# robotic-vision-lab/Edge-Informed-Contrast-Maximization

Hardware: AMD Instinct MI355X
Metric: warped-events/sec/GPU + loss+grad eval ms, 1e6 events @ 346x260 (higher is better)
Workload: dtype f32

## Files before the change

### edge-informed-contrast-maximization_amd/csrc/eincm_api.hip

```cpp
#include <hip/hip_runtime.h>
#include <hip/hip_ext.h>

#include <algorithm>
#include <chrono>
#include <cmath>
#include <cstdarg>
#include <cstdio>
#include <cstdlib>
#include <cstring>
#include <string>
#include <vector>

#include "eincm.h"
#include "eincm_kernels.hip.h"
#include "eincm_kernels_f64.hip.h"
#include "eincm_binning.hip.h"
#include "eincm_edges.hip.h"
#include "eincm_objectives.hip.h"
#include "eincm_splat_window.hip.h"
#include "eincm_canny.hip.h"
#include "eincm_preprocess.hip.h"
#include "eincm_gtflow.hip.h"

using namespace eincm;
// ... 1236 lines not shown
    if (n_in < 1 || n_out < 1 || !A || method < 0 || method > EINCM_METHOD_CUBIC) return EINCM_ERR_ARG;
    std::vector<double> M;
    resample_matrix(n_in, n_out, method, M);
    memcpy(A, M.data(), M.size() * sizeof(double));
    return EINCM_OK;
}

eincm_ctx* eincm_create(int device, int H, int W, int max_refs, int max_windows, int64_t max_events_total, uint32_t flags) {
    if (H < 3 || W < 3 || H > 32767 || W > 32767 || max_refs < 1 || max_refs > EINCM_MAX_REFS || max_windows < 1 ||
        max_events_total < 1 || max_events_total > (int64_t)2000000000) {
        fail(nullptr, EINCM_ERR_ARG, "eincm_create: bad argument (H=%d W=%d max_refs=%d max_windows=%d max_events=%lld)",
             H, W, max_refs, max_windows, (long long)max_events_total);
        return nullptr;
    }
    int ndev = 0;
    hipError_t e = hipGetDeviceCount(&ndev);
    if (e != hipSuccess || ndev < 1) {
        fail(nullptr, EINCM_ERR_HIP, "eincm_create: no HIP device visible (%s); this engine has no CPU fallback",
             hipGetErrorString(e));
        return nullptr;
    }
    if (device < 0 || device >= ndev) {
        fail(nullptr, EINCM_ERR_ARG, "eincm_create: device %d out of range (0..%d)", device, ndev - 1);
        return nullptr;
    }
    if ((flags & EINCM_CF_FP64) && (flags & (EINCM_CF_TIMING | EINCM_CF_TIMING_DOMINANT))) {
        fail(nullptr, EINCM_ERR_UNSUPPORTED, "eincm_create: the timing flags are not supported with EINCM_CF_FP64");
        return nullptr;
    }
    eincm_ctx* c = new eincm_ctx();
    c->fp64 = (flags & EINCM_CF_FP64) != 0;
    c->device = device; c->H = H; c->W = W; c->maxR = max_refs; c->maxB = max_windows; c->maxN = max_events_total;
    c->cflags = flags;
    if (const char* s = getenv("EINCM_SEG")) { int v = atoi(s); if (v >= 64 && v <= MAX_SEG) c->seg = v; }
    if (const char* s = getenv("EINCM_SEG_SPLAT")) { int v = atoi(s); if (v >= 64 && v <= MAX_CHUNK) c->seg_s = v; }
    if (const char* s = getenv("EINCM_WINCAP")) { int v = atoi(s); if (v >= 1024 && v <= 6912) { c->wincap = (v / 4) * 4; c->wincap_fixed = true; } }
    auto bail = [&](const char* what, hipError_t err) -> eincm_ctx* {
        fail(nullptr, EINCM_ERR_HIP, "eincm_create: %s failed: %s", what, hipGetErrorString(err));
        free_all(c);
        delete c;
        return nullptr;
    };
#define TRY(expr) do { hipError_t e2_ = (expr); if (e2_ != hipSuccess) return bail(#expr, e2_); } while (0)
    TRY(hipSetDevice(device));
    TRY(hipStreamCreateWithFlags(&c->stream, hipStreamNonBlocking));
    const int tilesX = (W + TS - 1) / TS, tilesY = (H + TS - 1) / TS, ntiles = tilesX * tilesY;
    const size_t B = max_windows, R = max_refs, img = (size_t)H * W;
    c->max_items = (int64_t)B * ntiles + max_events_total / 256 + 1;
    c->coarse_cap = 64 * 64 * 2;
    TRY(dalloc(&c->d_xy, (size_t)max_events_total));
    TRY(dalloc(&c->d_t, (size_t)max_events_total));
    TRY(dalloc(&c->d_xy_g, (size_t)max_events_total));
    TRY(dalloc(&c->d_t_g, (size_t)max_events_total));
    c->host_binning = (ntiles > BIN_MAX_TILES) || (getenv("EINCM_HOST_BINNING") != nullptr);
    for (SegList* L : {&c->gather, &c->splat, &c->splat_sh, &c->gather_2}) {
        TRY(dalloc(&L->d_items, (size_t)c->max_items));
        TRY(dalloc(&L->d_order, (size_t)c->max_items));
    }
    for (SegList* L : {&c->gather, &c->gather_2}) TRY(dalloc(&L->d_win_item0, B + 1));
    for (SegList* L : {&c->gather, &c->splat}) {
        TRY(dalloc(&L->d_wins, (size_t)c->max_items * max_refs));
        if (!c->host_binning) TRY(dalloc(&L->d_itembase, B * ntiles));
    }
    TRY(dalloc(&c->d_raw_x, (size_t)max_events_total));
    TRY(dalloc(&c->d_raw_y, (size_t)max_events_total));
    TRY(dalloc(&c->d_raw_t, (size_t)max_events_total));
    if (!c->host_binning) {
// ... 153 lines not shown
    if (c && c->pend.active && c->pend.launched)
        return fail(c, EINCM_ERR_STATE, "an asynchronous evaluation is in flight: call eincm_loss_grad_wait first");
    if (!c) return EINCM_ERR_ARG;
    if (n_windows < 1 || n_windows > c->maxB) return fail(c, EINCM_ERR_ARG, "n_windows %d outside 1..%d", n_windows, c->maxB);
    if (n_refs < 1 || n_refs > c->maxR) return fail(c, EINCM_ERR_ARG, "n_refs %d outside 1..%d", n_refs, c->maxR);
    if (!n_events || !xs_w || !ys_w || !ts_w || !edges_w || !edge_ts) return fail(c, EINCM_ERR_ARG, "null pointer argument");
    if (n_windows >= 1 && n_windows <= c->maxB)
        for (int b = 0; b < n_windows; ++b)
            if (!edges_w[b] || (n_events[b] > 0 && (!xs_w[b] || !ys_w[b] || !ts_w[b]))) return fail(c, EINCM_ERR_ARG, "null pointer argument (window %d)", b);
    HIPCHK(c, hipSetDevice(c->device));
    c->objc_valid = false;
    const int H = c->H, W = c->W;
    int64_t N = 0;
    for (int b = 0; b < n_windows; ++b) {
        if (n_events[b] < 0) return fail(c, EINCM_ERR_ARG, "n_events[%d] negative", b);
        N += n_events[b];
    }
    if (N > c->maxN) return fail(c, EINCM_ERR_ARG, "total events %lld exceed capacity %lld", (long long)N, (long long)c->maxN);
    c->staged = false;
    c->Theta_valid = false;
    struct DrainOnExit { hipStream_t s; ~DrainOnExit() { (void)hipStreamSynchronize(s); } } drain_on_exit{c->stream};
    if (c->acc_dirty) { const int rcd = clear_accumulators(c); if (rcd) return rcd; }
    Geom g{};
    g.H = H; g.W = W; g.R = n_refs; g.B = n_windows;
    g.tilesX = (W + TS - 1) / TS; g.tilesY = (H + TS - 1) / TS; g.ntiles = g.tilesX * g.tilesY;
    g.igx = (W + IG_COLS - 1) / IG_COLS; g.nig = g.igx * ((H + IG_ROWS - 1) / IG_ROWS);
    g.pstride = std::max(g.ntiles, NSPART);
    g.gmax_n = g.R * g.nig;
    g.wincap = c->wincap; g.winmaxw = win_maxw(c->wincap);
    g.wincap_a = g.wincap; g.winmaxw_a = g.winmaxw;

    const double x_wg = ((double)N / 8192.0 + 0.5 * n_windows * g.ntiles) * n_refs;
    int seg = c->seg > 0 ? c->seg : 16384;
    int seg_2 = (x_wg >= 4000.0 && (double)N / ((double)n_windows * g.ntiles) < 16384.0) ? 16384 : (x_wg < 1000.0 ? 4096 : 8192);
    if (const char* e = getenv("EINCM_SEG_2DOF")) { const int v = atoi(e); if (v >= 64 && v <= MAX_SEG) seg_2 = v; }
    const double per_tile = (double)N / ((double)n_windows * g.ntiles);
    int seg_s = c->seg_s > 0 ? c->seg_s : (x_wg >= 3000.0 && per_tile < 16384.0 ? 16384 : (x_wg >= 400.0 ? 8192 : 4096));
    g.pitch_aligned = (x_wg >= 3000.0 && per_tile < 16384.0) ? 1 : 0;
    if (const char* e = getenv("EINCM_PITCH_ALIGNED")) g.pitch_aligned = std::max(0, std::min(2, atoi(e)));
    const bool sort_segments = getenv("EINCM_NO_SEGSORT") == nullptr;
    const size_t img = (size_t)H * W;
    for (int b = 0; b < n_windows; ++b) {
        memset(&c->h_wc[b], 0, sizeof(WinConst));
        multi_ref_weights(n_refs, c->h_wc[b].mrw);
        for (int r = 0; r < n_refs; ++r)
            if (!std::isfinite(edge_ts[b * n_refs + r])) return fail(c, EINCM_ERR_ARG, "edge_ts[%d,%d] is not finite", b, r);
    }
    std::vector<unsigned> cntmax_h((size_t)n_windows, 0u);
    std::vector<double> dtmax_h((size_t)n_windows, 0.0);
    bool edge_ts_uploaded = false;
    int rc = EINCM_OK;
    auto copy_for_gather = [&]() -> int {
        if (c->gather.n == 0) return EINCM_OK;
        if (sort_segments) {
            hipLaunchKernelGGL(k_segsort, dim3(std::min(c->gather.n, 8192)), dim3(SORT_NT), 0, c->stream, c->gather.n, c->gather.d_items,
                               c->d_xy, c->d_t, c->d_xy_g, c->d_t_g);
            return EINCM_OK;
        }
        HIPCHK(c, hipMemcpyAsync(c->d_xy_g, c->d_xy, (size_t)N * sizeof(uint32_t), hipMemcpyDeviceToDevice, c->stream));
        HIPCHK(c, hipMemcpyAsync(c->d_t_g, c->d_t, (size_t)N * sizeof(double), hipMemcpyDeviceToDevice, c->stream));
        return EINCM_OK;
    };
    if (!c->host_binning) {
        std::vector<BinBlock> blks;
        std::vector<int32_t> win_blk((size_t)n_windows + 1);
        int64_t base = 0;
        for (int b = 0; b < n_windows; ++b) {
            win_blk[b] = (int32_t)blks.size();
            for (int64_t s0 = 0; s0 < n_events[b]; s0 += BIN_CHUNK) {
                BinBlock bb; bb.win = b; bb.start = (int32_t)(base + s0); bb.count = (int32_t)std::min<int64_t>(BIN_CHUNK, n_events[b] - s0);
                bb.first_blk = win_blk[b];
                blks.push_back(bb);
            }
            base += n_events[b];
        }
        win_blk[n_windows] = (int32_t)blks.size();
        const int nblk = (int)blks.size();
        if (nblk > c->max_binblocks) return fail(c, EINCM_ERR_ARG, "internal: %d staging blocks exceed capacity", nblk);
        int32_t misc_init[4] = {0, 0, 0x7fffffff, 0x7fffffff};
        HIPCHK(c, hipMemcpyAsync(c->d_bin_misc, misc_init, sizeof misc_init, hipMemcpyHostToDevice, c->stream));
        HIPCHK(c, hipMemcpyAsync(c->d_win_blk, win_blk.data(), win_blk.size() * sizeof(int32_t), hipMemcpyHostToDevice, c->stream));
        for (int b = 0; b < n_windows; ++b)
            HIPCHK(c, hipMemcpyAsync(c->d_edges_raw + (size_t)b * n_refs * img, edges_w[b], (size_t)n_refs * img * sizeof(double), hipMemcpyHostToDevice, c->stream));
        hipLaunchKernelGGL(k_edges, dim3(EDGE_PARTS, n_refs, n_windows), dim3(NT), 0, c->stream, g, c->d_edges_raw, c->d_edges, c->d_edge_moments);
        if (nblk > 0) {
            HIPCHK(c, hipMemcpyAsync(c->d_binblocks, blks.data(), blks.size() * sizeof(BinBlock), hipMemcpyHostToDevice, c->stream));
            int64_t off = 0;
            for (int b = 0; b < n_windows; ++b) {
                const size_t nb = (size_t)n_events[b];
                if (nb > 0) {
                    HIPCHK(c, hipMemcpyAsync(c->d_raw_x + off, xs_w[b], nb * sizeof(int16_t), hipMemcpyHostToDevice, c->stream));
                    HIPCHK(c, hipMemcpyAsync(c->d_raw_y + off, ys_w[b], nb * sizeof(int16_t), hipMemcpyHostToDevice, c->stream));
// ... 1121 lines not shown
```

### edge-informed-contrast-maximization_amd/csrc/eincm_binning.hip.h

```cpp
#pragma once
#include <hip/hip_runtime.h>
#include <stdint.h>

#include "eincm_kernels.hip.h"

namespace eincm {

constexpr int BIN_CHUNK = 1024;
constexpr int BIN_NT = 64;
constexpr int BIN_TRIPS = BIN_CHUNK / BIN_NT;
constexpr int BIN_MAX_TILES = 12288;

struct BinBlock { int32_t win, start, count, first_blk; };

__global__ __launch_bounds__(BIN_NT) void k_bin_hist(Geom g, const BinBlock* __restrict__ blks, const int16_t* __restrict__ xs,
                                                  const int16_t* __restrict__ ys, const double* __restrict__ ts,
                                                  uint32_t* __restrict__ blockhist, int* __restrict__ err)
{
    extern __shared__ uint32_t hist[];
    const BinBlock bb = blks[blockIdx.x];
    uint32_t xy[BIN_TRIPS]; double tt[BIN_TRIPS];
#pragma unroll
    for (int k = 0; k < BIN_TRIPS; ++k) {
        const int i = k * BIN_NT + (int)threadIdx.x;
// ... 119 lines not shown
    __shared__ __attribute__((aligned(16))) uint32_t keys[256];
    const int idx = blockIdx.x;
    const int cnt = tilecount[idx], base = tilebase[idx];
    const int t = threadIdx.x;
    for (int b0 = blockIdx.y * 256; b0 + 256 <= cnt; b0 += 256 * gridDim.y) {
        const uint32_t xy = ev_xy[base + b0 + t];
        const double tm = ev_t[base + b0 + t];
        const uint32_t key = (((xy & 31u) << 5) | ((xy >> 16) & 31u)) << 8 | (uint32_t)t;
        __syncthreads();
        keys[t] = key;
        __syncthreads();
        int rank = 0;
        const uint4* k4 = reinterpret_cast<const uint4*>(keys);
#pragma unroll 8
        for (int k = 0; k < 64; ++k) {
            const uint4 q = k4[k];
            rank += (q.x < key ? 1 : 0) + (q.y < key ? 1 : 0) + (q.z < key ? 1 : 0) + (q.w < key ? 1 : 0);
        }
        const int hw = rank & 7;
        const int pos = (hw >> 1) * 64 + (hw & 1) * 32 + (rank >> 3);
        ev_xy[base + b0 + pos] = xy;
        ev_t[base + b0 + pos] = tm;
    }
}

struct SegLayout {
    int n0, K0, K1, rem0, rem1;
    __host__ __device__ explicit SegLayout(int n) {
        n0 = (n + 1) >> 1;
        const int n1 = n - n0;
        K0 = (n0 + 255) >> 8; K1 = (n1 + 255) >> 8;
        rem0 = n0 - 256 * (K0 - 1); rem1 = n1 - 256 * (K1 - 1);
    }
    __host__ __device__ int position(int s) const {
        const int c = s >= n0;
        const int sc = c ? s - n0 : s, K = c ? K1 : K0, rem = c ? rem1 : rem0;
        int t, j;
        if (sc < rem * K) { t = sc / K; j = sc - t * K; }
        else { const int q = sc - rem * K; t = rem + q / (K - 1); j = q - (t - rem) * (K - 1); }
        return (c ? n0 : 0) + j * 256 + t;
    }
};
constexpr int SORT_NT = 256, SORT_NW = SORT_NT / 64, SORT_KEYS = TS * TS, SORT_KEY_BITS = 10;
static_assert(SORT_KEYS == 1 << SORT_KEY_BITS, "pixkey has SORT_KEY_BITS bits");
__device__ __forceinline__ uint32_t pixkey(uint32_t xy) { return ((xy >> 11) & (31u << 5)) | (xy & 31u); }
__global__ __launch_bounds__(SORT_NT) void k_segsort(int n_items, const Item* __restrict__ items,
                                                      const uint32_t* __restrict__ src_xy, const double* __restrict__ src_t,
                                                      uint32_t* __restrict__ dst_xy, double* __restrict__ dst_t)
{
    __shared__ uint32_t cnt[SORT_NW][SORT_KEYS];
    __shared__ uint32_t wsum[SORT_NT];
    const int lane = threadIdx.x & 63, wv = threadIdx.x >> 6;
    const unsigned long long lt_mask = (1ull << lane) - 1ull;
    for (int k = blockIdx.x; k < n_items; k += gridDim.x) {
        const Item it = items[k];
        const int n = it.count, begin = it.begin;
        const int qlen = (((n + SORT_NW - 1) / SORT_NW + 63) / 64) * 64;
        const int lo = min(wv * qlen, n), hi = min(lo + qlen, n);
        for (int i = threadIdx.x; i < SORT_NW * SORT_KEYS; i += SORT_NT) (&cnt[0][0])[i] = 0u;
        __syncthreads();
        for (int i = lo + lane; i < hi; i += 64) atomicAdd(&cnt[wv][pixkey(src_xy[begin + i])], 1u);
        __syncthreads();
        uint32_t c[4][SORT_NW], tot = 0u;
#pragma unroll
        for (int q = 0; q < 4; ++q)
#pragma unroll
            for (int w = 0; w < SORT_NW; ++w) { c[q][w] = cnt[w][4 * threadIdx.x + q]; tot += c[q][w]; }
        wsum[threadIdx.x] = tot;
        __syncthreads();
        for (int off = 1; off < SORT_NT; off <<= 1) {
            const uint32_t v = (threadIdx.x >= off) ? wsum[threadIdx.x - off] : 0u;
            __syncthreads();
            wsum[threadIdx.x] += v;
            __syncthreads();
        }
        uint32_t run = wsum[threadIdx.x] - tot;
#pragma unroll
        for (int q = 0; q < 4; ++q)
#pragma unroll
            for (int w = 0; w < SORT_NW; ++w) { cnt[w][4 * threadIdx.x + q] = run; run += c[q][w]; }
        __syncthreads();
        const SegLayout L(n);
        uint32_t nxy = 0u; double nt = 0.0;
        if (lo + lane < hi) { nxy = src_xy[begin + lo + lane]; nt = src_t[begin + lo + lane]; }
        for (int i0 = lo; i0 < hi; i0 += 64) {
            const int i = i0 + lane;
            const bool valid = i < hi;
            const uint32_t xy = nxy; const double t = nt;
            if (i + 64 < hi) { nxy = src_xy[begin + i + 64]; nt = src_t[begin + i + 64]; }
            const int key = valid ? (int)pixkey(xy) : -1;
            unsigned long long grp = __ballot(valid);
#pragma unroll
            for (int bit = 0; bit < SORT_KEY_BITS; ++bit) {
                const bool one = ((key >> bit) & 1) != 0;
                const unsigned long long bal = __ballot(one);
                grp &= one ? bal : ~bal;
            }
            uint32_t rank = 0u, base = 0u;
            if (valid) { base = cnt[wv][key]; rank = base + (uint32_t)__popcll(grp & lt_mask); }
            __builtin_amdgcn_wave_barrier();
            if (valid && (grp & lt_mask) == 0ull) cnt[wv][key] = base + (uint32_t)__popcll(grp);
            __builtin_amdgcn_wave_barrier();
            if (valid) {
                const int pos = L.position((int)rank);
                dst_xy[begin + pos] = xy;
                dst_t[begin + pos] = t;
            }
        }
        __syncthreads();
    }
}

__global__ void k_items(Geom g, int seg, const int32_t* __restrict__ tilecount, const int32_t* __restrict__ tilebase,
                        const int32_t* __restrict__ itembase, Item* __restrict__ items)
{
    const int idx = blockIdx.x * blockDim.x + threadIdx.x;
    if (idx >= g.B * g.ntiles) return;
    const int c = tilecount[idx], base = tilebase[idx];
    int k = itembase[idx];
    const int len = balanced_seg_len(c, seg);
    for (int s = 0; s < c; s += len, ++k) {
        Item it;
        it.win = idx / g.ntiles; it.tile = idx % g.ntiles; it.begin = base + s; it.count = min(len, c - s);
        it.t_lo = 0.0; it.t_hi = 0.0;
        items[k] = it;
    }
}

__global__ __launch_bounds__(NT) void k_seg_minmax(int n_items, Item* __restrict__ items, const double* __restrict__ ev_t)
{
    __shared__ double smn[NWAVE], smx[NWAVE];
    for (int k = blockIdx.x; k < n_items; k += gridDim.x) {
        const int begin = items[k].begin, count = items[k].count;
        double mn = INFINITY, mx = -INFINITY;
        for (int i = threadIdx.x; i < count; i += NT) { const double t = ev_t[begin + i]; mn = fmin(mn, t); mx = fmax(mx, t); }
        mn = wave_min(mn); mx = wave_max(mx);
        __syncthreads();
        if ((threadIdx.x & 63) == 0) { smn[threadIdx.x >> 6] = mn; smx[threadIdx.x >> 6] = mx; }
        __syncthreads();
        if (threadIdx.x == 0) {
            for (int i = 1; i < NWAVE; ++i) { mn = fmin(mn, smn[i]); mx = fmax(mx, smx[i]); }
            items[k].t_lo = mn; items[k].t_hi = mx;
        }
// ... 54 lines not shown
```

### edge-informed-contrast-maximization_amd/csrc/eincm_kernels.hip.h

```cpp
#pragma once
#include <hip/hip_runtime.h>
#include <stdint.h>

namespace eincm {

constexpr int TS = 32;
constexpr int NT = 256;
constexpr int NWAVE = NT / 64;
constexpr int WIN_CAP_DEFAULT = 2304;
constexpr int WIN_CAP_MAX = 9216;
constexpr int NXCD = 8;
constexpr double EPSN = 2.220446049250313e-16;
constexpr float INV_2PI = 0.15915494309189535f;
constexpr int MAX_CHUNK = 16384;
constexpr int MAX_SEG = 1 << 20;
__device__ __forceinline__ int fix_shift(int count) {
    const unsigned c = (unsigned)ceilf((float)count * 0.16f);
    const int ceillog2 = (c <= 1u) ? 0 : (32 - __clz(c - 1u));
    return min(30, 32 - ceillog2);
}
__host__ __device__ __forceinline__ int balanced_seg_len(int c, int seg) {
    const int nseg = (c + seg - 1) / seg;
    if (nseg <= 1) return seg;
    const int len = (((c + nseg - 1) / nseg + 255) / 256) * 256;
    return len < seg ? len : seg;
}
constexpr float EXP_M05 = 0.6065306597126334f;

struct Geom {
    int H, W, R, B;
    int tilesX, tilesY, ntiles;
    int wincap, winmaxw;
    int wincap_a, winmaxw_a;
    int nparts;
    int pstride;
    int gmax_n;
    unsigned long long wmask;
    int igx, nig;
    int pitch_aligned;
};

__device__ __forceinline__ bool win_active(const Geom& g, int b) { return b >= 64 || ((g.wmask >> b) & 1ull) != 0ull; }

struct Item {
    int32_t win, tile, begin, count;
    double t_lo, t_hi;
};

// ... 148 lines not shown
        const int nwh = min(wh, wincap / (aligned ? win_pitch(g, nww) : nww));
        bx0 = (bx0 + bx1) / 2 - nww / 2;
        by0 = (by0 + by1) / 2 - nwh / 2;
        ww = nww; wh = nwh;
    }
    Window w; w.ox = bx0; w.oy = by0; w.ww = ww; w.wh = wh;
    return w;
}

__device__ __forceinline__ void warp_axis(int x, double v, double dt, int& ir, float& f) {
#ifndef EINCM_ABL_WARP_FMA
#pragma clang fp contract(off)
#endif
    const double w = (double)x - v * dt;
    const double r = rint(w);
    f = (float)(w - r);
    ir = (int)r;
}
__device__ __forceinline__ int clamp_far(int ir) { return min(max(ir, -(1 << 20)), 1 << 20); }

struct f2v { float x, y; };

__device__ __forceinline__ void taps3x2(float fx, float fy, float scale_y, f2v& km, f2v& k0, f2v& kp) {
    constexpr float L2E = 1.4426950408889634f, EXP_M1 = 0.36787944117144233f;
    const float bx = __builtin_amdgcn_exp2f(fmaf(fx, L2E, -0.5f * L2E)), by = __builtin_amdgcn_exp2f(fmaf(fy, L2E, -0.5f * L2E));
    const float ax = EXP_M1 * __builtin_amdgcn_rcpf(bx), ay = EXP_M1 * __builtin_amdgcn_rcpf(by);
    const float s = __builtin_amdgcn_exp2f(fmaf(fx, fx, fy * fy) * (-0.5f * L2E)) * scale_y;
    km.x = ax; km.y = s * ay;
    k0.x = 1.0f; k0.y = s;
    kp.x = bx; kp.y = s * by;
}

struct EvReg { uint32_t xy; double t; };

constexpr int THETA_CONST = 1;
constexpr int THETA_TILE = 2;

__device__ __forceinline__ uint32_t cvt_rpi(float x) { uint32_t r; asm("v_cvt_rpi_i32_f32 %0, %1" : "=v"(r) : "v"(x)); return r; }
__device__ __forceinline__ uint32_t fix_u32(float a, float b) { return cvt_rpi(a * b); }

constexpr int RS_MAXC = 24;
struct TileRange { int ilo, ni, jlo, nj; };
struct ResampleTile {
    int ilo, ni, jlo, nj;
    bool staged;
};
struct ResampleLds {
    int2 rt[TS], ct[TS];
    double ah[TS * RS_MAXC], aw[TS * RS_MAXC];
    int rng[4];
};
__device__ __forceinline__ ResampleTile stage_resample_ranges(ResampleLds& L, int h, int w, int x0, int y0, int x1, int y1,
                                                              const int2* __restrict__ rowtap, const int2* __restrict__ coltap) {
    const int t = threadIdx.x;
    if (t < TS) L.rt[t] = (y0 + t < y1) ? rowtap[y0 + t] : make_int2(h, 0);
    else if (t < 2 * TS) L.ct[t - TS] = (x0 + t - TS < x1) ? coltap[x0 + t - TS] : make_int2(w, 0);
    __syncthreads();
    if (t < 64) {
        const int2 v = (t < TS) ? L.rt[t] : L.ct[t - TS];
        int lo = v.x, hi = v.y;
#pragma unroll
        for (int o = 16; o > 0; o >>= 1) { lo = min(lo, __shfl_xor(lo, o, 64)); hi = max(hi, __shfl_xor(hi, o, 64)); }
        if (t == 0) { L.rng[0] = lo; L.rng[1] = hi; }
        if (t == TS) { L.rng[2] = lo; L.rng[3] = hi; }
    }
    __syncthreads();
// ... 983 lines not shown
        }
    }
    if (!direct11) for (int i = threadIdx.x; i < TS * TS * 2; i += NTH) accum[i] = 0ull;
    auto G_at = [&](size_t p) -> float { return Gi[p]; };
    auto load_window = [&]() {
    if (wn.ox >= 0 && wn.oy >= 0 && wn.ox + wn.ww <= g.W && wn.oy + wn.wh <= g.H) {
        const size_t o0 = (size_t)wn.oy * g.W + wn.ox;
        for (WinWalkT<NTH> w(threadIdx.x, wn.ww); w.i < wn.ww * wn.wh; w.next()) lds[w.row * wp + w.col] = G_at(o0 + w.row * g.W + w.col);
    } else {
        for (int row = wv; row < wn.wh; row += NTH / 64) {
            const int gy = wrap_drop(wn.oy + row, g.H);
            for (int col = lane; col < wn.ww; col += 64) {
                const int gx = wrap_drop(wn.ox + col, g.W);
                lds[row * wp + col] = (gx >= 0 && gy >= 0) ? G_at((size_t)gy * g.W + gx) : 0.0f;
            }
        }
    }
    };
    load_window();
    double gscale = 0.0;
    double gm_used = 0.0;
    if (!direct11) {
        __shared__ unsigned gms[NTH / 64];
        const double gm = gmax_of(gmax + (size_t)it.win * g.gmax_n, g.gmax_n, gms);
        gscale = ldexp(1.0, grad_shift_pixel(wc[it.win], gm, g.R, WIDE != 0));
        gm_used = gm;
    }
    __syncthreads();

    const uint32_t* __restrict__ exy = ev_xy + it.begin;
    const double* __restrict__ et = ev_t + it.begin;
    const int n = it.count;
    const int tid = threadIdx.x;
    uint32_t cur_key = 0xffffffffu;
    double run_x = 0.0, run_y = 0.0;
    double2 vcur = vconst;
    auto flush_run = [&]() {
        if (cur_key == 0xffffffffu) return;
        unsigned long long* a = accum + (cur_key << 1);
        atomicAdd(a, (unsigned long long)(WIDE ? fix64_wide(run_x) : fix64(run_x)));
        atomicAdd(a + 1, (unsigned long long)(WIDE ? fix64_wide(run_y) : fix64(run_y)));
    };
    auto gather_ev = [&](const EvReg& ev) {
        const double dt = ev.t - tau;
        const int x = ev.xy & 0xffff, y = ev.xy >> 16;
        if (theta_mode != THETA_CONST) {
            const uint32_t key = ((ev.xy >> 11) & (31u << 5)) | (ev.xy & 31u);
#ifdef EINCM_ABL_G_NORUN
            vcur = thtile[key];
#else
            if (key != cur_key) {
                flush_run();
                cur_key = key; run_x = 0.0; run_y = 0.0;
                vcur = thtile[key];
            }
#endif
        }
        float gwx, gwy;
        event_dLdw(g, wn, wp, lds, G_at, x, y, vcur, dt, gwx, gwy);
        if (direct11) {
            const float ndt = (float)(-dt);
            f11x = fmaf(ndt, gwx, f11x); f11y = fmaf(ndt, gwy, f11y);
        } else {
            const double sdt = -dt * gscale;
            run_x = fma(sdt, (double)gwx, run_x); run_y = fma(sdt, (double)gwy, run_y);
        }
    };
    const SegWalk<NTH> walk(n, tid);
    auto walk_half = [&](int c) {
        const int K = c ? walk.K1 : walk.K0, rem = c ? walk.rem1 : walk.rem0;
        const uint32_t* __restrict__ px = exy + (c ? walk.n0 : 0) + walk.tt;
        const double* __restrict__ pt = et + (c ? walk.n0 : 0) + walk.tt;
#pragma unroll 2
        for (int j = 0; j < K - 1; ++j) {
            EvReg ev; ev.xy = px[j * 256]; ev.t = pt[j * 256];
            gather_ev(ev);
        }
        if (K > 0 && walk.tt < rem) {
            EvReg ev; ev.xy = px[(K - 1) * 256]; ev.t = pt[(K - 1) * 256];
            gather_ev(ev);
        }
    };
    for (int rr = r; ; ) {
#ifndef EINCM_ABL_G_NOEVENTS
    if (NTH == 512) walk_half(walk.half);
    else { walk_half(0); walk_half(1); }
    if (!direct11) { flush_run(); cur_key = 0xffffffffu; run_x = 0.0; run_y = 0.0; }
#endif
    if (!all_r || ++rr >= g.R) break;
    __syncthreads();
    tau = edge_ts[it.win * g.R + rr];
    wn = wins[(size_t)item * g.R + rr];
    wp = wn.ww;
    img = ((size_t)it.win * g.R + rr) * g.H * g.W;
    Gi = G + img;
    load_window();
    __syncthreads();
    }
    if (direct11) {
        double sum11x = block_sum<NTH / 64>((double)f11x, red11);
        double sum11y = block_sum<NTH / 64>((double)f11y, red11);
        if (threadIdx.x == 0) {
            double* dst = g11 + ((size_t)item * g.R + r) * 2;
            dst[0] = sum11x; dst[1] = sum11y;
        }
        return;
    }
    __syncthreads();
#ifdef EINCM_ABL_G_NOFLUSH
    return;
#endif
    if (PROJ) {
        const TileRange tr = tilerng[it.tile];
        static_assert(PROJ_SCRATCH_BYTES <= WIN_CAP_DEFAULT * 4, "the projection's scratch fits the smallest G window");
        const double gmd = gm_used;
        const double scale = ldexp(1.0, grad_shift(wc[it.win], gmd, g.R) - grad_shift_pixel(wc[it.win], gmd, g.R, WIDE != 0));
        for (int p = threadIdx.x; p < TS * TS; p += NTH) {
            const int ly = p >> 5, lx = p & 31;
            const long long vx = (long long)accum[p * 2], vy = (long long)accum[p * 2 + 1];
            thtile[(ly << 5) + (lx ^ ly)] = make_double2((double)vx * scale, (double)vy * scale);
// ... 566 lines not shown
```

### edge-informed-contrast-maximization_amd/csrc/eincm_kernels_f64.hip.h

```cpp
#pragma once
#include "eincm_kernels.hip.h"
#include <cfloat>

namespace eincm {

constexpr int F64_PIX = 2048;
constexpr int F64_PA = 3;
constexpr int F64_PB = 6;
constexpr int F64_PC = 2;
constexpr double INV_2PI_D = 0.15915494309189535;
constexpr double EXP_M1_D = 0.36787944117144233;

struct F64Scal {
    double m, M, D, cm, cM, mean, var, g2, mse, div;
};

template <typename Op>
__device__ __forceinline__ double block_reduce64(double v, double* scratch, Op op) {
#pragma unroll
    for (int o = 32; o > 0; o >>= 1) v = op(v, __shfl_down(v, o, 64));
    const int lane = threadIdx.x & 63, wv = threadIdx.x >> 6;
    __syncthreads();
    if (lane == 0) scratch[wv] = v;
    __syncthreads();
// ... 22 lines not shown
    k[1] = e0;
    k[2] = e0 * bp;
}

template <typename A>
__device__ __forceinline__ void scharr64(const A& a, int y, int x, double& gx, double& gy) {
    const double pp = a(y + 1, x + 1), pm = a(y + 1, x - 1), mp = a(y - 1, x + 1), mm = a(y - 1, x - 1);
    gx = 3.0 * (pp - pm) + 10.0 * (a(y, x + 1) - a(y, x - 1)) + 3.0 * (mp - mm);
    gy = 3.0 * (pp - mp) + 10.0 * (a(y + 1, x) - a(y - 1, x)) + 3.0 * (pm - mm);
}
__device__ __constant__ const double DIVK64[3][3] = {{1.0 / 12, 1.0 / 6, 1.0 / 12}, {1.0 / 6, 0.0, 1.0 / 6}, {1.0 / 12, 1.0 / 6, 1.0 / 12}};

constexpr int F64_WIN = 4096;

__global__ __launch_bounds__(NT) void k64_splat(Geom g, int n_items, const Item* __restrict__ items, const uint32_t* __restrict__ ev_xy,
                                                 const double* __restrict__ ev_t, const double* __restrict__ Theta,
                                                 const double* __restrict__ edge_ts, const int* __restrict__ ishift,
                                                 unsigned long long* __restrict__ acc)
{
    __shared__ unsigned long long win[F64_WIN];
    __shared__ double scratch[NWAVE];
    int item, r;
    if (!block_to_work(n_items, g.R, nullptr, item, r)) return;
    const Item it = items[item];
    if (!win_active(g, it.win)) return;
    const double tau = edge_ts[it.win * g.R + r];
    const double scale = ldexp(INV_2PI_D, ishift[it.win]);
    const double* __restrict__ Th = Theta + (size_t)it.win * g.H * g.W * 2;
    unsigned long long* __restrict__ img = acc + ((size_t)it.win * g.R + r) * g.H * g.W;
    double mnx = INFINITY, mxx = -INFINITY, mny = INFINITY, mxy = -INFINITY;
    for (int i = threadIdx.x; i < it.count; i += NT) {
        const uint32_t xy = ev_xy[it.begin + i];
        const double dt = ev_t[it.begin + i] - tau;
        const int x = xy & 0xffff, y = xy >> 16;
        const double2 v = *reinterpret_cast<const double2*>(Th + ((size_t)y * g.W + x) * 2);
        int irx, iry; double fx, fy;
        warp_axis64(x, v.x, dt, irx, fx);
        warp_axis64(y, v.y, dt, iry, fy);
        const double cx = (double)clamp_far(irx), cy = (double)clamp_far(iry);
        mnx = fmin(mnx, cx); mxx = fmax(mxx, cx); mny = fmin(mny, cy); mxy = fmax(mxy, cy);
    }
    mnx = block_reduce64(mnx, scratch, OpMin()); mxx = block_reduce64(mxx, scratch, OpMax());
    mny = block_reduce64(mny, scratch, OpMin()); mxy = block_reduce64(mxy, scratch, OpMax());
    if (!(mnx <= mxx)) return;
    const int ox = (int)fmax(mnx - 1.0, 0.0), ex = (int)fmin(mxx + 1.0, (double)(g.W - 1));
    const int oy = (int)fmax(mny - 1.0, 0.0), ey = (int)fmin(mxy + 1.0, (double)(g.H - 1));
    const int ww = ex - ox + 1, wh = ey - oy + 1;
    const bool use_lds = ww > 0 && wh > 0 && ww * wh <= F64_WIN;
    if (use_lds) {
        for (int k = threadIdx.x; k < ww * wh; k += NT) win[k] = 0ull;
        __syncthreads();
    }
    for (int i = threadIdx.x; i < it.count; i += NT) {
        const uint32_t xy = ev_xy[it.begin + i];
        const double dt = ev_t[it.begin + i] - tau;
        const int x = xy & 0xffff, y = xy >> 16;
        const double2 v = *reinterpret_cast<const double2*>(Th + ((size_t)y * g.W + x) * 2);
        int irx, iry; double fx, fy;
        warp_axis64(x, v.x, dt, irx, fx);
        warp_axis64(y, v.y, dt, iry, fy);
        const int cx = clamp_far(irx), cy = clamp_far(iry);
        double kx[3], ky[3];
        taps64(fx, kx);
        taps64(fy, ky);
#pragma unroll
        for (int dy = -1; dy <= 1; ++dy) {
            const int py = wrap_drop(cy + dy, g.H);
            if (py < 0) continue;
            const double sy = ky[dy + 1] * scale;
#pragma unroll
            for (int dx = -1; dx <= 1; ++dx) {
                const int px = wrap_drop(cx + dx, g.W);
                if (px < 0) continue;
                const unsigned long long q = (unsigned long long)rint(kx[dx + 1] * sy);
                const int lx = px - ox, ly = py - oy;
                if (use_lds && (unsigned)lx < (unsigned)ww && (unsigned)ly < (unsigned)wh) atomicAdd(&win[ly * ww + lx], q);
                else atomicAdd(img + (size_t)py * g.W + px, q);
            }
        }
    }
    if (use_lds) {
        __syncthreads();
        for (int k = threadIdx.x; k < ww * wh; k += NT) {
            const unsigned long long q = win[k];
            if (q) atomicAdd(img + (size_t)(oy + k / ww) * g.W + ox + k % ww, q);
        }
    }
}

// ... 244 lines not shown
    add_u128(p, lo, hi);
    return true;
}
__device__ __forceinline__ double i128_to_double(unsigned long long lo, unsigned long long hi) {
    const bool neg = (long long)hi < 0;
    if (neg) { lo = ~lo + 1ull; hi = ~hi + (lo == 0ull ? 1ull : 0ull); }
    const double v = (double)hi * 0x1p64 + (double)lo;
    return neg ? -v : v;
}

__global__ __launch_bounds__(NT) void k64_gather(Geom g, int n_items, const Item* __restrict__ items, const uint32_t* __restrict__ ev_xy,
                                                  const double* __restrict__ ev_t, const double* __restrict__ Theta,
                                                  const double* __restrict__ edge_ts, const double* __restrict__ G,
                                                  const WinConst* __restrict__ wcs, const unsigned long long* __restrict__ gmax,
                                                  unsigned long long* __restrict__ gacc , unsigned* __restrict__ bad)
{
    __shared__ unsigned long long lacc[TS * TS * 2 * 2];
    if ((int)blockIdx.x >= n_items) return;
    const Item it = items[blockIdx.x];
    const int b = it.win;
    if (!win_active(g, b)) return;
    const int tx0 = (it.tile % g.tilesX) * TS, ty0 = (it.tile / g.tilesX) * TS;
    for (int k = threadIdx.x; k < TS * TS * 4; k += NT) lacc[k] = 0ull;
    __syncthreads();
    bool flag = false;
    const int H = g.H, W = g.W, R = g.R;
    const size_t HW = (size_t)H * W;
    const double scale = ldexp(1.0, gshift64(wcs[b], gmax[b], R));
    const double* __restrict__ Th = Theta + (size_t)b * HW * 2;
    const double* __restrict__ Gb = G + (size_t)b * R * HW;
    for (int i = threadIdx.x; i < it.count; i += NT) {
        const uint32_t xy = ev_xy[it.begin + i];
        const double t = ev_t[it.begin + i];
        const int x = xy & 0xffff, y = xy >> 16;
        const double2 v = *reinterpret_cast<const double2*>(Th + ((size_t)y * W + x) * 2);
        double cx = 0.0, cy = 0.0;
        for (int r = 0; r < R; ++r) {
            const double dt = t - edge_ts[b * R + r];
            int irx, iry; double fx, fy;
            warp_axis64(x, v.x, dt, irx, fx);
            warp_axis64(y, v.y, dt, iry, fy);
            const int ix = clamp_far(irx), iy = clamp_far(iry);
            double kx[3], ky[3];
            taps64(fx, kx);
            taps64(fy, ky);
            const double* __restrict__ Gr = Gb + (size_t)r * HW;
            double sx = 0.0, sy = 0.0;
#pragma unroll
            for (int dy = -1; dy <= 1; ++dy) {
                const int py = wrap_drop(iy + dy, H);
                if (py < 0) continue;
#pragma unroll
                for (int dx = -1; dx <= 1; ++dx) {
                    const int px = wrap_drop(ix + dx, W);
                    if (px < 0) continue;
                    const double gk = Gr[(size_t)py * W + px] * (kx[dx + 1] * ky[dy + 1] * INV_2PI_D);
                    sx += gk * ((double)dx - fx);
                    sy += gk * ((double)dy - fy);
                }
            }
            cx += -dt * sx;
            cy += -dt * sy;
        }
        const int lx = x - tx0, ly = y - ty0;
        unsigned long long* a = ((unsigned)lx < (unsigned)TS && (unsigned)ly < (unsigned)TS) ? lacc + (ly * TS + lx) * 4
                                                                                            : gacc + (((size_t)b * HW + (size_t)y * W + x) * 2) * 2;
        const bool okx = add_i128(a, rint(cx * scale));
// ... 113 lines not shown
```

### edge-informed-contrast-maximization_amd/csrc/eincm_splat_window.hip.h

```cpp
#pragma once
#include "eincm_kernels.hip.h"

namespace eincm {

constexpr int SPLAT_RADIUS_MAX = 3;
constexpr int SW_CAP_TILE = 4608;
constexpr int SW_CAP_CONST = 6912;

__device__ __forceinline__ Window item_window_r(const Geom& g, const Item& it, const double* mm4, double tau, int wincap, int winmaxw, int rad) {
    const int tx = it.tile % g.tilesX, ty = it.tile / g.tilesX;
    const int x0 = tx * TS, y0 = ty * TS;
    const int x1 = min(x0 + TS, g.W) - 1, y1 = min(y0 + TS, g.H) - 1;
    const double dlo = it.t_lo - tau, dhi = it.t_hi - tau;
    const double LIM = 4096.0;
    double lo[2], hi[2];
#pragma unroll
    for (int c = 0; c < 2; ++c) {
        const double vmin = mm4[2 * c], vmax = mm4[2 * c + 1];
        const double a = -vmin * dlo, b = -vmin * dhi, cc = -vmax * dlo, d = -vmax * dhi;
        double mn = fmin(fmin(a, b), fmin(cc, d)), mx = fmax(fmax(a, b), fmax(cc, d));
        if (!(mn == mn) || !(mx == mx)) { mn = 0.0; mx = 0.0; }
        lo[c] = floor(fmin(fmax(mn, -LIM), LIM));
        hi[c] = ceil(fmin(fmax(mx, -LIM), LIM));
    }
// ... 135 lines not shown
    constexpr int K = 2 * RAD + 1;
    constexpr bool direct11 = TM == THETA_CONST;
    extern __shared__ __attribute__((aligned(16))) float lds[];
    __shared__ double red[NWAVE];
    __shared__ unsigned gms[NWAVE];
    unsigned long long* accum = reinterpret_cast<unsigned long long*>(lds + g.wincap_a);
    double2* thtile = reinterpret_cast<double2*>(lds + g.wincap_a + TS * TS * 4);
    int item, r;
    if (!block_to_work(n_items, g.R, nullptr, item, r)) return;
    const Item it = items[item];
    if (!win_active(g, it.win)) return;
    const double tau = edge_ts[it.win * g.R + r];
    double mm4[4];
    const double2 vconst = window_velocity<TM>(g, it, use_arg, theta_c, targ, tmm, mm4);
    const Window wn = item_window_r(g, it, mm4, tau, g.wincap_a, g.winmaxw_a, RAD);
    const float* __restrict__ Gi = G + ((size_t)it.win * g.R + r) * g.H * g.W;
    const int x0 = (it.tile % g.tilesX) * TS, y0 = (it.tile / g.tilesX) * TS;
    if (!direct11) {
        stage_theta_tile(g, it, Theta, thtile);
        for (int i = threadIdx.x; i < TS * TS * 2; i += NT) accum[i] = 0ull;
    }
    for (WinWalk w(threadIdx.x, wn.ww); w.i < wn.ww * wn.wh; w.next()) {
        const int gx = wrap_drop(wn.ox + w.col, g.W), gy = wrap_drop(wn.oy + w.row, g.H);
        lds[w.i] = (gx >= 0 && gy >= 0) ? Gi[(size_t)gy * g.W + gx] : 0.0f;
    }
    double gscale = 0.0;
    if (!direct11) gscale = ldexp(1.0, grad_shift_pixel(wc[it.win], gmax_of(gmax + (size_t)it.win * g.gmax_n, g.gmax_n, gms), g.R, wide != 0));
    __syncthreads();

    float f11x = 0.0f, f11y = 0.0f;
    for (int e = threadIdx.x; e < it.count; e += NT) {
        const uint32_t xy = ev_xy[it.begin + e];
        const double dt = ev_t[it.begin + e] - tau;
        const int x = xy & 0xffff, y = xy >> 16;
        const uint32_t key = ((xy >> 11) & (31u << 5)) | (xy & 31u);
        const double2 v = direct11 ? vconst : thtile[key];
        int irx, iry; float fx, fy;
        warp_axis(x, v.x, dt, irx, fx);
        warp_axis(y, v.y, dt, iry, fy);
        float kx[K], ky[K];
        taps_axis<RAD>(fx, kx);
        taps_axis<RAD>(fy, ky);
        const int sx = clamp_far(irx), sy = clamp_far(iry);
        const int lx0 = sx - RAD - wn.ox, ly0 = sy - RAD - wn.oy;
        const bool inside = lx0 >= 0 && ly0 >= 0 && lx0 + K <= wn.ww && ly0 + K <= wn.wh;
        float c[K];
#pragma unroll
        for (int d = 0; d < K; ++d) c[d] = 0.0f;
        float gy_acc = 0.0f;
#pragma unroll
        for (int dy = 0; dy < K; ++dy) {
            float rr = 0.0f;
#pragma unroll
            for (int dx = 0; dx < K; ++dx) {
                float gv;
                if (inside) {
                    gv = lds[(ly0 + dy) * wn.ww + lx0 + dx];
                } else {
                    const int cx = lx0 + dx, cy = ly0 + dy;
                    if (cx >= 0 && cy >= 0 && cx < wn.ww && cy < wn.wh) {
                        gv = lds[cy * wn.ww + cx];
                    } else {
                        const int gx = wrap_drop(sx - RAD + dx, g.W), gy = wrap_drop(sy - RAD + dy, g.H);
                        gv = (gx >= 0 && gy >= 0) ? Gi[(size_t)gy * g.W + gx] : 0.0f;
                    }
                }
                rr = fmaf(kx[dx], gv, rr);
// ... 40 lines not shown
```

Measured before the change: 180.0 billion.

## Mark per-key run ends at sort time and accumulate gather runs in fp32

The segment sort now sets a RUN_END bit in each event's packed xy word on the last event of a thread's same-key run. The gather kernel uses that flag to decide when to flush, instead of recomputing and comparing keys. In the narrow (non-WIDE) path, run sums accumulate in fp32 and are scaled by gscale only at flush, and an explicit software-prefetch loop replaces the unrolled walk. It also adds a segment-size bound that keeps fp32 run length limited, and a copy kernel that sets the flag when sorting is off. The cost is a small precision change and a reserved high bit of y.

```diff
diff --git a/edge-informed-contrast-maximization_amd/csrc/eincm_api.hip b/edge-informed-contrast-maximization_amd/csrc/eincm_api.hip
--- a/edge-informed-contrast-maximization_amd/csrc/eincm_api.hip
+++ b/edge-informed-contrast-maximization_amd/csrc/eincm_api.hip
@@ -1292,7 +1292,7 @@
     c->fp64 = (flags & EINCM_CF_FP64) != 0;
     c->device = device; c->H = H; c->W = W; c->maxR = max_refs; c->maxB = max_windows; c->maxN = max_events_total;
     c->cflags = flags;
-    if (const char* s = getenv("EINCM_SEG")) { int v = atoi(s); if (v >= 64 && v <= MAX_SEG) c->seg = v; }
+    if (const char* s = getenv("EINCM_SEG")) { int v = atoi(s); if (v >= 64 && v <= GATHER_SEG_MAX) c->seg = v; }
     if (const char* s = getenv("EINCM_SEG_SPLAT")) { int v = atoi(s); if (v >= 64 && v <= MAX_CHUNK) c->seg_s = v; }
     if (const char* s = getenv("EINCM_WINCAP")) { int v = atoi(s); if (v >= 1024 && v <= 6912) { c->wincap = (v / 4) * 4; c->wincap_fixed = true; } }
     auto bail = [&](const char* what, hipError_t err) -> eincm_ctx* {
@@ -1512,6 +1512,8 @@
 
     const double x_wg = ((double)N / 8192.0 + 0.5 * n_windows * g.ntiles) * n_refs;
     int seg = c->seg > 0 ? c->seg : 16384;
+    if (gather_thread_terms(seg, 256) > RUN_F32_MAX_TERMS)
+        return fail(c, EINCM_ERR_ARG, "internal: gather segments of %d events exceed k_gather's fp32 run bound", seg);
     int seg_2 = (x_wg >= 4000.0 && (double)N / ((double)n_windows * g.ntiles) < 16384.0) ? 16384 : (x_wg < 1000.0 ? 4096 : 8192);
     if (const char* e = getenv("EINCM_SEG_2DOF")) { const int v = atoi(e); if (v >= 64 && v <= MAX_SEG) seg_2 = v; }
     const double per_tile = (double)N / ((double)n_windows * g.ntiles);
@@ -1537,7 +1539,8 @@
                                c->d_xy, c->d_t, c->d_xy_g, c->d_t_g);
             return EINCM_OK;
         }
-        HIPCHK(c, hipMemcpyAsync(c->d_xy_g, c->d_xy, (size_t)N * sizeof(uint32_t), hipMemcpyDeviceToDevice, c->stream));
+        hipLaunchKernelGGL(k_copy_runs, dim3((unsigned)std::min<int64_t>(((int64_t)N + NT - 1) / NT, 8192)), dim3(NT), 0, c->stream,
+                           (long long)N, c->d_xy, c->d_xy_g);
         HIPCHK(c, hipMemcpyAsync(c->d_t_g, c->d_t, (size_t)N * sizeof(double), hipMemcpyDeviceToDevice, c->stream));
         return EINCM_OK;
     };
diff --git a/edge-informed-contrast-maximization_amd/csrc/eincm_binning.hip.h b/edge-informed-contrast-maximization_amd/csrc/eincm_binning.hip.h
--- a/edge-informed-contrast-maximization_amd/csrc/eincm_binning.hip.h
+++ b/edge-informed-contrast-maximization_amd/csrc/eincm_binning.hip.h
@@ -175,12 +175,13 @@
         K0 = (n0 + 255) >> 8; K1 = (n1 + 255) >> 8;
         rem0 = n0 - 256 * (K0 - 1); rem1 = n1 - 256 * (K1 - 1);
     }
-    __host__ __device__ int position(int s) const {
+    __host__ __device__ int position(int s) const { bool last; return position(s, last); }
+    __host__ __device__ int position(int s, bool& last) const {
         const int c = s >= n0;
         const int sc = c ? s - n0 : s, K = c ? K1 : K0, rem = c ? rem1 : rem0;
         int t, j;
-        if (sc < rem * K) { t = sc / K; j = sc - t * K; }
-        else { const int q = sc - rem * K; t = rem + q / (K - 1); j = q - (t - rem) * (K - 1); }
+        if (sc < rem * K) { t = sc / K; j = sc - t * K; last = j == K - 1; }
+        else { const int q = sc - rem * K; t = rem + q / (K - 1); j = q - (t - rem) * (K - 1); last = j == K - 2; }
         return (c ? n0 : 0) + j * 256 + t;
     }
 };
@@ -193,6 +194,7 @@
 {
     __shared__ uint32_t cnt[SORT_NW][SORT_KEYS];
     __shared__ uint32_t wsum[SORT_NT];
+    __shared__ uint32_t kend[SORT_KEYS];
     const int lane = threadIdx.x & 63, wv = threadIdx.x >> 6;
     const unsigned long long lt_mask = (1ull << lane) - 1ull;
     for (int k = blockIdx.x; k < n_items; k += gridDim.x) {
@@ -219,9 +221,11 @@
         }
         uint32_t run = wsum[threadIdx.x] - tot;
 #pragma unroll
-        for (int q = 0; q < 4; ++q)
+        for (int q = 0; q < 4; ++q) {
 #pragma unroll
             for (int w = 0; w < SORT_NW; ++w) { cnt[w][4 * threadIdx.x + q] = run; run += c[q][w]; }
+            kend[4 * threadIdx.x + q] = run;
+        }
         __syncthreads();
         const SegLayout L(n);
         uint32_t nxy = 0u; double nt = 0.0;
@@ -245,13 +249,19 @@
             if (valid && (grp & lt_mask) == 0ull) cnt[wv][key] = base + (uint32_t)__popcll(grp);
             __builtin_amdgcn_wave_barrier();
             if (valid) {
-                const int pos = L.position((int)rank);
-                dst_xy[begin + pos] = xy;
+                bool last;
+                const int pos = L.position((int)rank, last);
+                dst_xy[begin + pos] = xy | ((last || rank + 1u == kend[key]) ? RUN_END : 0u);
                 dst_t[begin + pos] = t;
             }
         }
         __syncthreads();
     }
+}
+
+__global__ __launch_bounds__(NT) void k_copy_runs(long long n, const uint32_t* __restrict__ src_xy, uint32_t* __restrict__ dst_xy)
+{
+    for (long long i = (long long)blockIdx.x * NT + threadIdx.x; i < n; i += (long long)gridDim.x * NT) dst_xy[i] = src_xy[i] | RUN_END;
 }
 
 __global__ void k_items(Geom g, int seg, const int32_t* __restrict__ tilecount, const int32_t* __restrict__ tilebase,
diff --git a/edge-informed-contrast-maximization_amd/csrc/eincm_kernels.hip.h b/edge-informed-contrast-maximization_amd/csrc/eincm_kernels.hip.h
--- a/edge-informed-contrast-maximization_amd/csrc/eincm_kernels.hip.h
+++ b/edge-informed-contrast-maximization_amd/csrc/eincm_kernels.hip.h
@@ -1,6 +1,7 @@
 #pragma once
 #include <hip/hip_runtime.h>
 #include <stdint.h>
+#include <type_traits>
 
 namespace eincm {
 
@@ -14,6 +15,10 @@
 constexpr float INV_2PI = 0.15915494309189535f;
 constexpr int MAX_CHUNK = 16384;
 constexpr int MAX_SEG = 1 << 20;
+constexpr int RUN_F32_MAX_TERMS = 64;
+__host__ __device__ constexpr int gather_thread_terms(int seg, int nth) { return (nth == 512 ? 1 : 2) * (((seg + 1) / 2 + 255) / 256); }
+constexpr int GATHER_SEG_MAX = 16384;
+static_assert(gather_thread_terms(GATHER_SEG_MAX, 256) <= RUN_F32_MAX_TERMS, "k_gather's fp32 run sums outgrow their bound");
 __device__ __forceinline__ int fix_shift(int count) {
     const unsigned c = (unsigned)ceilf((float)count * 0.16f);
     const int ceillog2 = (c <= 1u) ? 0 : (32 - __clz(c - 1u));
@@ -228,6 +233,9 @@
 }
 
 struct EvReg { uint32_t xy; double t; };
+
+constexpr uint32_t RUN_END = 0x80000000u;
+__host__ __device__ __forceinline__ int ev_y(uint32_t xy) { return (int)((xy >> 16) & 0x7fffu); }
 
 constexpr int THETA_CONST = 1;
 constexpr int THETA_TILE = 2;
@@ -1277,28 +1285,36 @@
     const double* __restrict__ et = ev_t + it.begin;
     const int n = it.count;
     const int tid = threadIdx.x;
+    using RunT = typename std::conditional<WIDE != 0, double, float>::type;
     uint32_t cur_key = 0xffffffffu;
-    double run_x = 0.0, run_y = 0.0;
+    bool opens = true;
+    RunT run_x = 0, run_y = 0;
     double2 vcur = vconst;
     auto flush_run = [&]() {
         if (cur_key == 0xffffffffu) return;
         unsigned long long* a = accum + (cur_key << 1);
-        atomicAdd(a, (unsigned long long)(WIDE ? fix64_wide(run_x) : fix64(run_x)));
-        atomicAdd(a + 1, (unsigned long long)(WIDE ? fix64_wide(run_y) : fix64(run_y)));
+        if (WIDE) {
+            atomicAdd(a, (unsigned long long)fix64_wide((double)run_x));
+            atomicAdd(a + 1, (unsigned long long)fix64_wide((double)run_y));
+        } else {
+            atomicAdd(a, (unsigned long long)fix64((double)run_x * gscale));
+            atomicAdd(a + 1, (unsigned long long)fix64((double)run_y * gscale));
+        }
     };
     auto gather_ev = [&](const EvReg& ev) {
         const double dt = ev.t - tau;
-        const int x = ev.xy & 0xffff, y = ev.xy >> 16;
+        const int x = ev.xy & 0xffff, y = ev_y(ev.xy);
         if (theta_mode != THETA_CONST) {
-            const uint32_t key = ((ev.xy >> 11) & (31u << 5)) | (ev.xy & 31u);
 #ifdef EINCM_ABL_G_NORUN
-            vcur = thtile[key];
+            vcur = thtile[((ev.xy >> 11) & (31u << 5)) | (ev.xy & 31u)];
 #else
-            if (key != cur_key) {
+            if (opens) {
                 flush_run();
-                cur_key = key; run_x = 0.0; run_y = 0.0;
-                vcur = thtile[key];
-            }
+                cur_key = ((ev.xy >> 11) & (31u << 5)) | (ev.xy & 31u);
+                run_x = 0; run_y = 0;
+                vcur = thtile[cur_key];
+            }
+            opens = (ev.xy & RUN_END) != 0u;
 #endif
         }
         float gwx, gwy;
@@ -1306,9 +1322,12 @@
         if (direct11) {
             const float ndt = (float)(-dt);
             f11x = fmaf(ndt, gwx, f11x); f11y = fmaf(ndt, gwy, f11y);
+        } else if (WIDE) {
+            const double sdt = -dt * gscale;
+            run_x = fma(sdt, (double)gwx, (double)run_x); run_y = fma(sdt, (double)gwy, (double)run_y);
         } else {
-            const double sdt = -dt * gscale;
-            run_x = fma(sdt, (double)gwx, run_x); run_y = fma(sdt, (double)gwy, run_y);
+            const float ndt = (float)(-dt);
+            run_x = fmaf(ndt, gwx, (float)run_x); run_y = fmaf(ndt, gwy, (float)run_y);
         }
     };
     const SegWalk<NTH> walk(n, tid);
@@ -1316,6 +1335,17 @@
         const int K = c ? walk.K1 : walk.K0, rem = c ? walk.rem1 : walk.rem0;
         const uint32_t* __restrict__ px = exy + (c ? walk.n0 : 0) + walk.tt;
         const double* __restrict__ pt = et + (c ? walk.n0 : 0) + walk.tt;
+        if (!direct11) {
+            const int cnt = K > 0 ? K - 1 + (walk.tt < rem ? 1 : 0) : 0;
+            if (cnt == 0) return;
+            EvReg nx; nx.xy = px[0]; nx.t = pt[0];
+            for (int j = 0; j < cnt; ++j) {
+                const EvReg ev = nx;
+                if (j + 1 < cnt) { nx.xy = px[(j + 1) * 256]; nx.t = pt[(j + 1) * 256]; }
+                gather_ev(ev);
+            }
+            return;
+        }
 #pragma unroll 2
         for (int j = 0; j < K - 1; ++j) {
             EvReg ev; ev.xy = px[j * 256]; ev.t = pt[j * 256];
@@ -1330,7 +1360,7 @@
 #ifndef EINCM_ABL_G_NOEVENTS
     if (NTH == 512) walk_half(walk.half);
     else { walk_half(0); walk_half(1); }
-    if (!direct11) { flush_run(); cur_key = 0xffffffffu; run_x = 0.0; run_y = 0.0; }
+    if (!direct11) { flush_run(); cur_key = 0xffffffffu; opens = true; run_x = 0; run_y = 0; }
 #endif
     if (!all_r || ++rr >= g.R) break;
     __syncthreads();
diff --git a/edge-informed-contrast-maximization_amd/csrc/eincm_kernels_f64.hip.h b/edge-informed-contrast-maximization_amd/csrc/eincm_kernels_f64.hip.h
--- a/edge-informed-contrast-maximization_amd/csrc/eincm_kernels_f64.hip.h
+++ b/edge-informed-contrast-maximization_amd/csrc/eincm_kernels_f64.hip.h
@@ -78,7 +78,7 @@
     for (int i = threadIdx.x; i < it.count; i += NT) {
         const uint32_t xy = ev_xy[it.begin + i];
         const double dt = ev_t[it.begin + i] - tau;
-        const int x = xy & 0xffff, y = xy >> 16;
+        const int x = xy & 0xffff, y = ev_y(xy);
         const double2 v = *reinterpret_cast<const double2*>(Th + ((size_t)y * g.W + x) * 2);
         int irx, iry; double fx, fy;
         warp_axis64(x, v.x, dt, irx, fx);
@@ -100,7 +100,7 @@
     for (int i = threadIdx.x; i < it.count; i += NT) {
         const uint32_t xy = ev_xy[it.begin + i];
         const double dt = ev_t[it.begin + i] - tau;
-        const int x = xy & 0xffff, y = xy >> 16;
+        const int x = xy & 0xffff, y = ev_y(xy);
         const double2 v = *reinterpret_cast<const double2*>(Th + ((size_t)y * g.W + x) * 2);
         int irx, iry; double fx, fy;
         warp_axis64(x, v.x, dt, irx, fx);
@@ -411,7 +411,7 @@
     for (int i = threadIdx.x; i < it.count; i += NT) {
         const uint32_t xy = ev_xy[it.begin + i];
         const double t = ev_t[it.begin + i];
-        const int x = xy & 0xffff, y = xy >> 16;
+        const int x = xy & 0xffff, y = ev_y(xy);
         const double2 v = *reinterpret_cast<const double2*>(Th + ((size_t)y * W + x) * 2);
         double cx = 0.0, cy = 0.0;
         for (int r = 0; r < R; ++r) {
diff --git a/edge-informed-contrast-maximization_amd/csrc/eincm_splat_window.hip.h b/edge-informed-contrast-maximization_amd/csrc/eincm_splat_window.hip.h
--- a/edge-informed-contrast-maximization_amd/csrc/eincm_splat_window.hip.h
+++ b/edge-informed-contrast-maximization_amd/csrc/eincm_splat_window.hip.h
@@ -191,7 +191,7 @@
     for (int e = threadIdx.x; e < it.count; e += NT) {
         const uint32_t xy = ev_xy[it.begin + e];
         const double dt = ev_t[it.begin + e] - tau;
-        const int x = xy & 0xffff, y = xy >> 16;
+        const int x = xy & 0xffff, y = ev_y(xy);
         const uint32_t key = ((xy >> 11) & (31u << 5)) | (xy & 31u);
         const double2 v = direct11 ? vconst : thtile[key];
         int irx, iry; float fx, fy;
```

After: 179.8 billion (median of 3 runs). No clear change (-0.1%).
